# KRLGroup/gym-ma-survival-2d

Measured on NVIDIA B200. Metric: agent_steps_per_sec, higher is better.
Workload: dtype f32

## Files before the change

### gym-ma-survival-2d_b200/csrc/msv_abi.cu

```cuda
#include <cuda_runtime.h>
#include <math.h>
#include <stdio.h>
#include <stdlib.h>
#include <string.h>
#include <string>
#include <vector>
#include <map>
#include <algorithm>

#include "../../include/masurv.h"
#include "msv_launch.h"

extern "C" {
typedef struct { int32_t device_type; int32_t device_id; } DLDevice;
typedef struct { uint8_t code; uint8_t bits; uint16_t lanes; } DLDataType;
typedef struct {
  void* data; DLDevice device; int32_t ndim; DLDataType dtype;
  int64_t* shape; int64_t* strides; uint64_t byte_offset;
} DLTensor;
typedef struct DLManagedTensor {
  DLTensor dl_tensor; void* manager_ctx; void (*deleter)(struct DLManagedTensor*);
} DLManagedTensor;
}

// ... 1035 lines not shown
    const int64_t wr = 76 * A + 32 + 32 + 24 * PW + 16 + 8 + om + 4 * A + 1;
    return rd + wr;
  }
  if (which == 1) return 48 * A + 8 + om + 16 + 32 * B + 16 * B + 8 * H + 40 + (int64_t)h->obs.n_elems * 4;
  if (which == 2) return L > 0 ? 16 + 32 * B + 16 * B + 8 * H + 32 * A + 8 * A * L : 0;
  return 0;
}
int64_t msv_bytes_per_env_step(msv_handle* h) {
  return msv_kernel_bytes_per_env(h, 0) + msv_kernel_bytes_per_env(h, 1) + msv_kernel_bytes_per_env(h, 2);
}
int64_t msv_obs_bytes_per_env(msv_handle* h) { return h ? (int64_t)h->obs.n_elems * 4 : 0; }
int64_t msv_kernel_launches(msv_handle* h) { return h ? h->launches : 0; }
int msv_tile_plan(msv_handle* h, int32_t out[4]) {
  if (!h || !out) return MSV_ERR_INVALID;
  out[0] = h->C.epb; out[1] = h->C.N / h->C.epb; out[2] = h->C.epb * h->AC; out[3] = (h->handoff && h->cfg.auto_reset != 2) ? 1 : 0;
  return MSV_OK;
}

int msv_debug_profile(msv_handle* h, int enable, unsigned long long out[64]) {
  if (!h) return MSV_ERR_INVALID;
  DevGuard g(h->device); CK(cudaDeviceSynchronize());
  if (out) CK(msv_read_profile(out, 1));
  h->C.profile = enable;
  return MSV_OK;
}

int msv_debug_blocks(msv_handle* h, unsigned long long* out, int n_words) {
  if (!h || !out) return MSV_ERR_INVALID;
  DevGuard g(h->device); CK(cudaDeviceSynchronize());
  CK(msv_read_blocks(out, n_words));
  return MSV_OK;
}

int msv_debug_trace(msv_handle* h, unsigned long long* out, int n_words) {
  if (!h || !out) return MSV_ERR_INVALID;
  DevGuard g(h->device); CK(cudaDeviceSynchronize());
  CK(msv_read_trace(out, n_words));
  return MSV_OK;
}

void msv_philox4x32(const uint32_t ctr[4], const uint32_t key[2], uint32_t out[4]) {
  uint32_t c0 = ctr[0], c1 = ctr[1], c2 = ctr[2], c3 = ctr[3], k0 = key[0], k1 = key[1];
  for (int r = 0; r < 10; ++r) {
    uint64_t p0 = (uint64_t)0xD2511F53u * c0, p1 = (uint64_t)0xCD9E8D57u * c2;
    uint32_t n0 = (uint32_t)(p1 >> 32) ^ c1 ^ k0, n1 = (uint32_t)p1, n2 = (uint32_t)(p0 >> 32) ^ c3 ^ k1, n3 = (uint32_t)p0;
    c0 = n0; c1 = n1; c2 = n2; c3 = n3; k0 += 0x9E3779B9u; k1 += 0xBB67AE85u;
  }
  out[0] = c0; out[1] = c1; out[2] = c2; out[3] = c3;
}

}
```

### gym-ma-survival-2d_b200/csrc/msv_device.cuh

```cuda
#pragma once
#include <cuda_runtime.h>
#include <stdint.h>
#include <float.h>

#define DEV __device__ __forceinline__

#define B2_PI 3.14159265359f
#define B2_EPS FLT_EPSILON
#define B2_LINEAR_SLOP 0.005f
#define B2_POLY_RADIUS (2.0f * B2_LINEAR_SLOP)
#define B2_AABB_EXT 0.1f
#define B2_AABB_MULT 2.0f
#define B2_VEL_THRESHOLD 1.0f
#define B2_MAX_LIN_CORR 0.2f
#define B2_MAX_TRANSLATION 2.0f
#define B2_MAX_ROTATION (0.5f * B2_PI)
#define B2_BAUMGARTE 0.2f
#define B2_TOI_BAUMGARTE 0.75f
#define B2_TIME_TO_SLEEP 0.5f
#define B2_LIN_SLEEP_TOL 0.01f
#define B2_ANG_SLEEP_TOL (2.0f / 180.0f * B2_PI)
#define B2_MAX_SUBSTEPS 8

struct f2 { float x, y; };
// ... 290 lines not shown
  r.px = (1.0f - beta) * A.px + beta * A.px;
  r.py = (1.0f - beta) * A.py + beta * A.py;
  if (A.ang != 0.0f) {
    float angle = (1.0f - beta) * A.ang + beta * A.ang;
    if (angle != A.ang) rot_set(angle, r.qs, r.qc);
  }
  return r;
}
DEV f2 point_at(f2 c0, f2 c, float beta) { return vadd(vmul(1.0f - beta, c0), vmul(beta, c)); }

#define TOI_FAILED 1
#define TOI_OVERLAPPED 2
#define TOI_TOUCHING 3
#define TOI_SEPARATED 4

#ifdef MSV_CHECK
__device__ unsigned long long g_chk[2];
#define CHK(cond) do { if (!(cond)) { atomicAdd(&g_chk[0], 1ull); g_chk[1] = __LINE__; } } while (0)
__device__ __forceinline__ int chk_idx_(int i, int n, int line) {
  if ((unsigned)i < (unsigned)n) return i;
  atomicAdd(&g_chk[0], 1ull); g_chk[1] = (unsigned long long)line;
  return 0;
}
#define CHK_IDX(i, n) chk_idx_((i), (n), __LINE__)
#else
#define CHK(cond) do { } while (0)
#define CHK_IDX(i, n) (i)
#endif
#ifdef MSV_PROFILE
__device__ unsigned long long g_dbg[8];
__device__ unsigned long long g_cnt[16];
__device__ unsigned long long g_sub[16];
__device__ unsigned long long g_toi[16];
#define TOIPROF(x) x
#define SUB_BEGIN() long long sub_t_ = clock64()
#define SUB(k) do { long long n_ = clock64(); atomicAdd(&g_sub[k], (unsigned long long)(n_ - sub_t_)); sub_t_ = n_; } while (0)
#define SUBCNT(k, v) atomicAdd(&g_sub[k], (unsigned long long)(v))
#define SUBMAX(k, tag) atomicMax(&g_sub[k], ((unsigned long long)(clock64() - sub_t_) << 8) | (unsigned long long)((tag) & 255))
#define RARE_BEGIN() long long rare_t0_ = clock64()
#define RARE_END(k) do { atomicAdd(&g_cnt[2 * (k)], 1ull); atomicAdd(&g_cnt[2 * (k) + 1], (unsigned long long)(clock64() - rare_t0_)); } while (0)
#else
#define RARE_BEGIN() do { } while (0)
#define RARE_END(k) do { } while (0)
#define SUB_BEGIN() do { } while (0)
#define SUB(k) do { } while (0)
#define SUBCNT(k, v) do { } while (0)
#define SUBMAX(k, tag) do { } while (0)
#define TOIPROF(x)
#endif
struct ToiOut { int state; float t; };
__device__ __noinline__ ToiOut time_of_impact_v(const SBox A, f2 c0, f2 c, float rB) {
  int state = 0; float tOut = 1.0f;
  const float tMax = 1.0f;
#ifdef MSV_PROFILE
  long long dbg_t0 = clock64(); int dbg_roots = 0, dbg_push = 0;
#endif
  float totalRadius = B2_POLY_RADIUS + rB;
  float target = fmax_(B2_LINEAR_SLOP, totalRadius - 3.0f * B2_LINEAR_SLOP);
  float tolerance = 0.25f * B2_LINEAR_SLOP;
  float t1 = 0.0f;
  int iter = 0;
  {
    f2 l = sb_mulT(A, c0);
    float dx = fmax_(fabsf(l.x) - A.hx, 0.0f), dy = fmax_(fabsf(l.y) - A.hy, 0.0f);
    float d = sqrtf(dx * dx + dy * dy);
    if (d > 1e-3f && d < (target + tolerance) - 1e-3f) { ToiOut r0; r0.state = TOI_TOUCHING; r0.t = 0.0f; return r0; }
  }
  SimplexCache cache; cache.count = 0;
  for (;;) {
    const float t1_in = t1; const SimplexCache cache_in = cache;
    SBox xfA = box_at(A, t1); f2 pB = point_at(c0, c, t1);
    float distance = gjk_distance(cache, xfA, pB);
    if (distance <= 0.0f) { state = TOI_OVERLAPPED; tOut = 0.0f; break; }
    if (distance < target + tolerance) { state = TOI_TOUCHING; tOut = t1; break; }
    int ftype; f2 axis, localPoint = mk2(0.0f, 0.0f); int ptIndexA = 0;
    if (cache.count == 1) {
      ftype = 0; ptIndexA = cache.indexA[0];
      f2 pointA = sb_mul(xfA, sb_vert(xfA, cache.indexA[0]));
      axis = vsub(pB, pointA); vnormalize(axis);
    } else {
      ftype = 1;
      f2 lA1 = sb_vert(xfA, cache.indexA[0]), lA2 = sb_vert(xfA, cache.indexA[1]);
      axis = cross_vs(vsub(lA2, lA1), 1.0f); vnormalize(axis);
      f2 normal = qmul(xfA.qs, xfA.qc, axis);
      localPoint = vmul(0.5f, vadd(lA1, lA2));
      f2 pointA = sb_mul(xfA, localPoint);
      float s = vdot(vsub(pB, pointA), normal);
      if (s < 0.0f) axis = vneg(axis);
    }
    (void)ptIndexA;
    bool done = false;
    float t2 = tMax;
    int pushBackIter = 0;
    for (;;) {
      int indexA = -1; float s2;
      {
        SBox x2 = box_at(A, t2); f2 p2 = point_at(c0, c, t2);
        if (ftype == 0) {
          indexA = box_support(x2, qmulT(x2.qs, x2.qc, axis));
          f2 pointA = sb_mul(x2, sb_vert(x2, indexA));
          s2 = vdot(vsub(p2, pointA), axis);
        } else {
          f2 normal = qmul(x2.qs, x2.qc, axis);
          f2 pointA = sb_mul(x2, localPoint);
          s2 = vdot(vsub(p2, pointA), normal);
        }
      }
      if (s2 > target + tolerance) { state = TOI_SEPARATED; tOut = tMax; done = true; break; }
      if (s2 > target - tolerance) { t1 = t2; break; }
      auto evaluate = [&](float t) -> float {
        SBox xt = box_at(A, t); f2 pt = point_at(c0, c, t);
        if (ftype == 0) {
          f2 pointA = sb_mul(xt, sb_vert(xt, indexA));
          return vdot(vsub(pt, pointA), axis);
        }
        f2 normal = qmul(xt.qs, xt.qc, axis);
        f2 pointA = sb_mul(xt, localPoint);
        return vdot(vsub(pt, pointA), normal);
      };
      float s1 = evaluate(t1);
      if (s1 < target - tolerance) { state = TOI_FAILED; tOut = t1; done = true; break; }
      if (s1 <= target + tolerance) { state = TOI_TOUCHING; tOut = t1; done = true; break; }
      int rootIterCount = 0;
      float a1 = t1, a2 = t2;
      for (;;) {
        float t;
        if (rootIterCount & 1) t = a1 + (target - s1) * (a2 - a1) / (s2 - s1);
        else t = 0.5f * (a1 + a2);
        ++rootIterCount;
#ifdef MSV_PROFILE
        ++dbg_roots;
#endif
        float s = evaluate(t);
        if (fabsf(s - target) < tolerance) { t2 = t; break; }
        if (s > target) { a1 = t; s1 = s; } else { a2 = t; s2 = s; }
        if (rootIterCount == 50) break;
      }
      ++pushBackIter;
#ifdef MSV_PROFILE
      ++dbg_push;
#endif
      if (pushBackIter == 8) break;
    }
    ++iter;
    if (done) break;
    if (iter == 20) { state = TOI_FAILED; tOut = t1; break; }
    if (t1 == t1_in && cache.count == cache_in.count && cache.metric == cache_in.metric &&
        cache.indexA[0] == cache_in.indexA[0] && (cache.count < 2 || cache.indexA[1] == cache_in.indexA[1]) &&
        (cache.count < 3 || cache.indexA[2] == cache_in.indexA[2])) {
      state = TOI_FAILED; tOut = t1; break;
    }
  }
#ifdef MSV_PROFILE
  atomicAdd(&g_dbg[0], 1ull); atomicMax(&g_dbg[1], (unsigned long long)iter); atomicMax(&g_dbg[2], (unsigned long long)dbg_roots);
  atomicMax(&g_dbg[3], (unsigned long long)dbg_push); atomicMax(&g_dbg[4], (unsigned long long)(clock64() - dbg_t0));
  atomicAdd(&g_dbg[5], (unsigned long long)(clock64() - dbg_t0));
#endif
  ToiOut r; r.state = state; r.t = tOut;
  return r;
}
DEV int time_of_impact(const SBox& A, f2 c0, f2 c, float rB, float& tOut) {
  ToiOut r = time_of_impact_v(A, c0, c, rB);
  tOut = r.t; return r.state;
}

DEV void philox4x32(uint32_t c0, uint32_t c1, uint32_t c2, uint32_t c3,
                    uint32_t k0, uint32_t k1, uint32_t out[4]) {
#pragma unroll
  for (int r = 0; r < 10; ++r) {
    uint32_t hi0 = __umulhi(0xD2511F53u, c0), lo0 = 0xD2511F53u * c0;
    uint32_t hi1 = __umulhi(0xCD9E8D57u, c2), lo1 = 0xCD9E8D57u * c2;
    uint32_t n0 = hi1 ^ c1 ^ k0, n1 = lo1, n2 = hi0 ^ c3 ^ k1, n3 = lo0;
    c0 = n0; c1 = n1; c2 = n2; c3 = n3;
    k0 += 0x9E3779B9u; k1 += 0xBB67AE85u;
  }
  out[0] = c0; out[1] = c1; out[2] = c2; out[3] = c3;
}
```

### gym-ma-survival-2d_b200/csrc/msv_env.cuh

```cuda
#pragma once
#include "msv_device.cuh"
#include "msv_types.cuh"
#include "msv_launch.h"

enum { F_CX, F_CY, F_A, F_VX, F_VY, F_W, F_C0X, F_C0Y, F_A0, F_ALPHA0, F_SLEEP,
       F_FAT0, F_FAT1, F_FAT2, F_FAT3, F_FLAGS, F_QS, F_QC, F_COUNT };
enum { G_X, G_Y, G_HX, G_HY, G_AX, G_AY, G_ROT, G_F0, G_F1, G_F2, G_F3, G_COUNT };
enum { K_META, K_SEQ, K_MTYPE, K_LNX, K_LNY, K_LPX, K_LPY, K_NI, K_TI, K_NM, K_TM, K_COUNT };
enum { KS_NX = K_SEQ, KS_NY = K_MTYPE, KS_PX = K_LNX, KS_PY = K_LNY, KS_RBX = K_LPX, KS_RBY = K_LPY };

#define FL_ALIVE 1
#define FL_AWAKE 2
#define FL_ISLAND 4
#define FL_MOVED 8

#define KIND_NONE 0
#define KIND_AGENT 1
#define KIND_BOX 2
#define KIND_ITEM 3
#define KIND_HEAL 4
#define KIND_WALL 5

#define STREAM_SHUFFLE 0
#define STREAM_BOX 1
#define STREAM_ZONE 2
#define STREAM_DEATH 3

template <int AC, int BC> struct PairLayout {
  static constexpr int NAA = AC * (AC - 1) / 2;
  static constexpr int NAB = AC * BC;
  static constexpr int P = NAA + NAB + AC * 4;
  static constexpr int PW = (P + 63) / 64;
};

struct TCon {
  int p, seq;
  int a;
  int sid;
  int b;
  int flags;
  Manifold m;
  float ni, ti;
  f2 normal, rA, rB;
  float normalMass, tangentMass;
};

struct BodyS { f2 c; float a; f2 v; float w; float invM, invI; };

extern __shared__ float msv_sm[];


#ifndef MSV_INLINE_MASK
#define MSV_INLINE_MASK 0
#endif
#ifndef MSV_TOI_COOP
#define MSV_TOI_COOP 0
#endif
#ifndef MSV_FIXPOINT
#define MSV_FIXPOINT 1
#endif
#if (MSV_INLINE_MASK >> 0) & 1
#define COLD0 __device__ __forceinline__
#else
#define COLD0 __device__ __noinline__
#endif
#if (MSV_INLINE_MASK >> 1) & 1
#define COLD1 __device__ __forceinline__
#else
#define COLD1 __device__ __noinline__
#endif
#if (MSV_INLINE_MASK >> 2) & 1
#define COLD2 __device__ __forceinline__
#else
#define COLD2 __device__ __noinline__
#endif
#if (MSV_INLINE_MASK >> 3) & 1
#define COLD3 __device__ __forceinline__
#else
#define COLD3 __device__ __noinline__
#endif
#if (MSV_INLINE_MASK >> 4) & 1
#define COLD4 __device__ __forceinline__
#else
#define COLD4 __device__ __noinline__
#endif

__device__ __noinline__ double2 philox_uniform2_of(const DevConst& C, uint32_t genv, uint32_t episode, uint32_t step, uint32_t stream, uint32_t blk) {
  uint32_t o[4];
  philox4x32(genv, episode, step, (stream << 16) | blk, C.seed_lo, C.seed_hi, o);
// ... 31 lines not shown
    rec[MSV_SP_BOX + 4 * b + 2] = hx; rec[MSV_SP_BOX + 4 * b + 3] = hy;
  }
  for (int h = 0; h < C.H0; ++h) { const int cell = perm[--top]; rec[MSV_SP_HEAL + 2 * h] = C.grid_px[cell]; rec[MSV_SP_HEAL + 2 * h + 1] = C.grid_py[cell]; }
  for (int i = 0; i < C.A; ++i) { const int cell = perm[--top]; rec[MSV_SP_AGENT + 2 * i] = C.grid_px[cell]; rec[MSV_SP_AGENT + 2 * i + 1] = C.grid_py[cell]; }
  if (C.zone_centers_random) {
    int d = 0;
    for (int z = C.n_zones - 1; z >= 0; --z) {
      const double L = C.floor_size - 2 * C.zone_radiuses[z];
      const double2 uz = philox_uniform2_of(C, genv, episode, 0u, STREAM_ZONE, (uint32_t)(d >> 1)); d += 2;
      rec[MSV_SP_ZONE + 2 * z] = (float)((uz.x * L) - L / 2); rec[MSV_SP_ZONE + 2 * z + 1] = (float)((uz.y * L) - L / 2);
    }
  } else {
    for (int z = 0; z < C.n_zones; ++z) { rec[MSV_SP_ZONE + 2 * z] = (float)C.zone_centers[z][0]; rec[MSV_SP_ZONE + 2 * z + 1] = (float)C.zone_centers[z][1]; }
  }
}

template <int AC, int BC, int HC, int G>
struct Env {
  using PL = PairLayout<AC, BC>;
  static constexpr int P = PL::P, PW = PL::PW, NAA = PL::NAA;
  static constexpr int MAXC = AC <= 4 ? 16 : 24;
  enum { L_HEALTH = 0, L_CAUSE = L_HEALTH + AC, L_COOLDOWN = L_CAUSE + AC, L_INV = L_COOLDOWN + AC,
         L_SREW = L_INV + AC, L_SKILLS = L_SREW + AC, L_SEENA = L_SKILLS + AC, L_SEENX = L_SEENA + AC,
         L_KCAUSE = L_SEENX + AC, L_EPRET = L_KCAUSE + AC,
         L_NP = L_EPRET + AC, L_STEPS, L_EPISODE, L_BODYSEQ, L_CONTACTSEQ, L_FIRST, L_OVERFLOW, L_NEWFIX,
         L_ZX, L_ZY, L_ZR, L_ZPHASE, L_ZTCOOL, L_ZTSHRINK, L_ZEND,
         L_STSTEPS, L_STHEALS, L_STBOXES, L_STEPISODES, L_USEHEAL, L_USEBOX, L_NEWBOX,
         L_PREALIVE, L_DMASK, L_NKILLS, L_COUNT };
  static constexpr int SLOTS = AC / G;
  static constexpr int W_BOX = F_COUNT * AC, W_TC = W_BOX + G_COUNT * BC, W_MISC = W_TC + K_COUNT * MAXC;
  static constexpr int W_ITEM = W_MISC + 2, W_HEAL = W_ITEM + 2 * BC;
  static constexpr int W_LEAD = W_HEAL + 2 * HC;
  static constexpr int W_TOI = W_LEAD + L_COUNT;
  static constexpr int SM_USED = W_TOI + AC * (BC + 4);
  static constexpr int SM_WORDS = SM_USED + ((G - SM_USED % 32) + 32) % 32;
  static constexpr int NR = 3;
  static_assert(AC % G == 0 && G <= 32 && (G & (G - 1)) == 0, "G must be a power of two dividing AC");

  const DevConst& C;
  const DevState& S;
  int es, g, e, N;
  int sb;
  unsigned gmask;
  bool lead;

  int nb, ni, nh;
  unsigned long long ex[PW], tc[PW], en[PW];
  unsigned long long own[PW];
  int ntc;

  __device__ __forceinline__ Env(const DevConst& c, const DevState& s, int es_, int g_, unsigned gmask_, int e_)
      : C(c), S(s), es(es_), g(g_), e(e_), N(c.N), sb(es_ * SM_WORDS), gmask(gmask_), lead(g_ == 0) {
#pragma unroll
    for (int w = 0; w < PW; ++w) own[w] = 0ull;
    for (int i = g; i < AC; i += G) {
      for (int a = 0; a < i; ++a) setb(own, p_aa(a, i));
      for (int k = 0; k < BC; ++k) setb(own, p_ab(i, k));
      for (int k = 0; k < 4; ++k) setb(own, p_aw(i, k));
    }
  }

  DEV void gsync() const { __syncwarp(gmask); }
  template <class V> DEV V bc(V v) const { return __shfl_sync(gmask, v, 0, G); }
  template <class V> DEV V from(V v, int j) const { return __shfl_sync(gmask, v, j, G); }
  DEV unsigned or32(unsigned v) const {
#pragma unroll
    for (int o = 1; o < G; o <<= 1) v |= __shfl_xor_sync(gmask, v, o, G);
    return v;
// ... 7 lines not shown
  DEV void share_bits() {
#pragma unroll
    for (int w = 0; w < PW; ++w) { ex[w] = bc(ex[w]); tc[w] = bc(tc[w]); en[w] = bc(en[w]); }
  }
  DEV void merge_bits() {
#pragma unroll
    for (int w = 0; w < PW; ++w) { ex[w] = or64(ex[w] & own[w]); tc[w] = or64(tc[w] & own[w]); en[w] = or64(en[w] & own[w]); }
  }

  DEV void take(const Env& o) {
    nb = o.nb; ni = o.ni; nh = o.nh; ntc = o.ntc;
#pragma unroll
    for (int w = 0; w < PW; ++w) { ex[w] = o.ex[w]; tc[w] = o.tc[w]; en[w] = o.en[w]; }
  }
#define MSV_COLD(call) do { Env c_(*this); c_.call; take(c_); } while (0)
#ifndef MSV_INLINE_MASK
#define MSV_INLINE_MASK 0
#endif
#define MSV_COLDK(k, call) do { if ((MSV_INLINE_MASK >> (k)) & 1) { call; } else { Env c_(*this); c_.call; take(c_); } } while (0)

  DEV float& AG(int f, int i) { return msv_sm[sb + (CHK_IDX(f, F_COUNT) * AC + CHK_IDX(i, AC))]; }
  DEV int& AGF(int i) { return reinterpret_cast<int*>(msv_sm)[sb + (F_FLAGS * AC + CHK_IDX(i, AC))]; }
  DEV float& BX(int f, int k) { return msv_sm[sb + (W_BOX + CHK_IDX(f, G_COUNT) * BC + CHK_IDX(k, BC))]; }
  DEV int& BXROT(int k) { return reinterpret_cast<int*>(msv_sm)[sb + (W_BOX + G_ROT * BC + CHK_IDX(k, BC))]; }
  DEV float& KF(int f, int k) { return msv_sm[sb + (W_TC + CHK_IDX(f, K_COUNT) * MAXC + CHK_IDX(k, MAXC))]; }
  DEV int& KI(int f, int k) { return reinterpret_cast<int*>(msv_sm)[sb + (W_TC + CHK_IDX(f, K_COUNT) * MAXC + CHK_IDX(k, MAXC))]; }
  DEV int& NTC() { return reinterpret_cast<int*>(msv_sm)[sb + (W_MISC + 0)]; }
  DEV float& ITP(int c, int k) { return msv_sm[sb + (W_ITEM + CHK_IDX(c, 2) * BC + CHK_IDX(k, BC))]; }
  DEV float& HLP(int c, int k) { return msv_sm[sb + (W_HEAL + CHK_IDX(c, 2) * HC + CHK_IDX(k, HC))]; }
  DEV int& LI(int k) { return reinterpret_cast<int*>(msv_sm)[sb + (W_LEAD + CHK_IDX(k, L_COUNT))]; }
  DEV unsigned& LU(int k) { return reinterpret_cast<unsigned*>(msv_sm)[sb + (W_LEAD + CHK_IDX(k, L_COUNT))]; }
  DEV float& LF(int k) { return msv_sm[sb + (W_LEAD + CHK_IDX(k, L_COUNT))]; }
  DEV float& TOIA(int i, int k) { return msv_sm[sb + (W_TOI + CHK_IDX(i, AC) * (BC + 4) + CHK_IDX(k, BC + 4))]; }
  DEV int& OVF() { return reinterpret_cast<int*>(msv_sm)[sb + (W_MISC + 1)]; }
  DEV bool alive(int i) { return AGF(i) & FL_ALIVE; }
  DEV bool awake(int i) { return AGF(i) & FL_AWAKE; }
  DEV f2 apos(int i) { return mk2(AG(F_CX, i), AG(F_CY, i)); }
  DEV static int meta_pack(int p, int a, int sid, int b) { return p | ((a + 1) << 8) | ((sid < 0 ? 0 : sid) << 12) | (b << 16); }
  DEV static void meta_unpack(int m, int& p, int& a, int& sid, int& b) { p = m & 255; a = ((m >> 8) & 15) - 1; sid = (m >> 12) & 15; b = (m >> 16) & 15; }

  DEV static bool bit(const unsigned long long* m, int p) {
    unsigned long long w = m[0];
#pragma unroll
    for (int q = 1; q < PW; ++q) if ((p >> 6) == q) w = m[q];
    return (w >> (p & 63)) & 1ull;
  }
  DEV static void setb(unsigned long long* m, int p) {
#pragma unroll
    for (int q = 0; q < PW; ++q) if (PW == 1 || (p >> 6) == q) m[q] |= 1ull << (p & 63);
  }
  DEV static void clrb(unsigned long long* m, int p) {
#pragma unroll
    for (int q = 0; q < PW; ++q) if (PW == 1 || (p >> 6) == q) m[q] &= ~(1ull << (p & 63));
  }
  DEV static int p_aa(int i, int j) { return j * (j - 1) / 2 + i; }
  DEV static int p_ab(int i, int k) { return NAA + i * BC + k; }
  DEV static int p_aw(int i, int k) { return NAA + AC * BC + i * 4 + k; }
  DEV static void decode(int p, int& a, int& sid, int& b) {
    CHK((unsigned)p < (unsigned)P);
    if (p < NAA) {
      int j = 1; while (j * (j + 1) / 2 <= p) ++j;
      a = p - j * (j - 1) / 2; b = j; sid = -1;
    } else if (p < NAA + AC * BC) {
      int q = p - NAA; a = -1; b = q / BC; sid = q % BC;
    } else {
      int q = p - NAA - AC * BC; a = -1; b = q >> 2; sid = BC + (q & 3);
// ... 1140 lines not shown
        const f2 v_in = vB; const float w_in = wB; bool changed = false;
        for (int k = 0; k < nisl; ++k) {
          const float ni0 = KF(K_NI, k), ti0 = KF(K_TI, k);
          float ni_ = ni0, ti_ = ti0;
          solve_velocity_static(mk2(KF(KS_NX, k), KF(KS_NY, k)), mk2(KF(KS_RBX, k), KF(KS_RBY, k)), KF(K_NM, k), KF(K_TM, k), ni_, ti_, vB, wB);
          KF(K_NI, k) = ni_; KF(K_TI, k) = ti_;
          changed |= __float_as_uint(ni_) != __float_as_uint(ni0) || __float_as_uint(ti_) != __float_as_uint(ti0);
        }
        if (!changed && __float_as_uint(vB.x) == __float_as_uint(v_in.x) && __float_as_uint(vB.y) == __float_as_uint(v_in.y) &&
            __float_as_uint(wB) == __float_as_uint(w_in)) break;
      }
      AG(F_VX, b) = vB.x; AG(F_VY, b) = vB.y; AG(F_W, b) = wB;
    }
    SUB(3);
    integrate_position(b, subdt);
    AGF(b) &= ~FL_MOVED;
    synchronize_fixtures(b);
    if (AGF(b) & FL_MOVED) find_new_contacts_of(b);
    SUB(4);
    bool same = prevP == minP;
    auto snap = [&](int q, unsigned v) { if (SNAP(q) != v) same = false; SNAP(q) = v; };
    for (int f = 0; f < F_COUNT; ++f) snap(f, __float_as_uint(AG(f, b)));
#pragma unroll
    for (int w = 0; w < PW; ++w) {
      snap(F_COUNT + 6 * w + 0, (unsigned)ex[w]); snap(F_COUNT + 6 * w + 1, (unsigned)(ex[w] >> 32));
      snap(F_COUNT + 6 * w + 2, (unsigned)tc[w]); snap(F_COUNT + 6 * w + 3, (unsigned)(tc[w] >> 32));
      snap(F_COUNT + 6 * w + 4, (unsigned)en[w]); snap(F_COUNT + 6 * w + 5, (unsigned)(en[w] >> 32));
    }
    snap(SNAPW - 1, (unsigned)LI(L_CONTACTSEQ));
    SUB(5);
    return 1 | (same ? 2 : 0);
  }

  DEV void solve_toi(float dt) {
    static_assert(SLOTS == 1, "solve_toi: one agent per lane");
    const int i = g;
    if (i < C.A) { AGF(i) &= ~FL_ISLAND; AG(F_ALPHA0, i) = 0.0f; }
    unsigned long long evcnt = 0ull; unsigned cvalid = 0u;
    int prevP = -1;
    auto toi_alpha = [&](int j, int k) {
      const SBox sbx = static_box(k);
      const f2 q0 = mk2(AG(F_C0X, j), AG(F_C0Y, j)), q1 = apos(j);
      float beta = 1.0f;
      const int state = time_of_impact(sbx, q0, q1, C.agent_r, beta);
      const float alpha0 = AG(F_ALPHA0, j);
      return state == TOI_TOUCHING ? fmin_(alpha0 + (1.0f - alpha0) * beta, 1.0f) : 1.0f;
    };
    TOIPROF(long long tp0 = clock64(); long long tp_ev = 0; int tp_it = 0; int tp_ran = 0; int tp_not = 0; int tp_same = 0; int tp_calls = 0;)
    for (int guard = 0; guard < 64; ++guard) {
      TOIPROF(tp_it++;)
      unsigned need = 0u;
      int minP = -1, minSeq = -1; float minAlpha = 1.0f;
      auto consider = [&](int p, float alpha) {
        if (alpha < 1.0f) {
          const int sq = (int)S.pseq[p * N + e];
          if (alpha < minAlpha || (alpha == minAlpha && sq > minSeq)) { minAlpha = alpha; minP = p; minSeq = sq; }
        }
      };
      if (i < C.A && alive(i) && awake(i)) {
#pragma unroll
        for (int w = 0; w < PW; ++w) {
          unsigned long long mbits = ex[w] & en[w] & own[w];
          if (w == 0) mbits &= ~((1ull << NAA) - 1ull);
          while (mbits) {
            int p = w * 64 + __ffsll((long long)mbits) - 1; mbits &= mbits - 1;
            int a_, k, i_; decode(p, a_, k, i_);
            const int cnt = (int)((evcnt >> (4 * k)) & 15ull);
            if (cnt > C.toi_max_count) continue;
            if ((cvalid >> k) & 1u) { consider(p, TOIA(i, k)); continue; }
            const SBox sbx = static_box(k);
            const f2 l0 = sb_mulT(sbx, mk2(AG(F_C0X, i), AG(F_C0Y, i))), l1 = sb_mulT(sbx, apos(i));
            const float gx = fmax_(fmin_(l0.x, l1.x) - sbx.hx, -sbx.hx - fmax_(l0.x, l1.x));
            const float gy = fmax_(fmin_(l0.y, l1.y) - sbx.hy, -sbx.hy - fmax_(l0.y, l1.y));
            if (fmax_(gx, gy) > (B2_POLY_RADIUS + C.agent_r - 3.0f * B2_LINEAR_SLOP) + 0.25f * B2_LINEAR_SLOP + 0.004f) { TOIA(i, k) = 1.0f; cvalid |= 1u << k; }
            else if (MSV_TOI_COOP) need |= 1u << k;
            else { const float al = toi_alpha(i, k); TOIA(i, k) = al; cvalid |= 1u << k; consider(p, al); }
          }
        }
      }
      if (MSV_TOI_COOP && __any_sync(gmask, need != 0u)) {
        unsigned ms[G]; int T = 0;
#pragma unroll
        for (int j = 0; j < G; ++j) { ms[j] = from(need, j); T += __popc(ms[j]); }
        TOIPROF(tp_calls += T;)
        for (int r0 = 0; r0 < T; r0 += G) {
          const int t = r0 + g;
          int fj = -1, fk = 0, base = 0;
#pragma unroll
          for (int j = 0; j < G; ++j) {
            const int c = __popc(ms[j]);
            if (t >= base && t < base + c) { fj = j; fk = (int)__fns(ms[j], 0u, t - base + 1); }
            base += c;
          }
          if (fj >= 0) TOIA(fj, fk) = toi_alpha(fj, fk);
        }
        gsync();
        cvalid |= need;
        while (need) {
          const int k = __ffs((int)need) - 1; need &= need - 1u;
          consider(k < BC ? p_ab(i, k) : p_aw(i, k - BC), TOIA(i, k));
        }
      }
#pragma unroll
      for (int o = 1; o < G; o <<= 1) {
        float oa = __shfl_xor_sync(gmask, minAlpha, o, G);
        int op = __shfl_xor_sync(gmask, minP, o, G), os = __shfl_xor_sync(gmask, minSeq, o, G);
        if (op >= 0 && (oa < minAlpha || (oa == minAlpha && os > minSeq))) { minAlpha = oa; minP = op; minSeq = os; }
      }
      if (minP < 0 || 1.0f - 10.0f * B2_EPS < minAlpha) break;
      int ea, ek, eb; decode(minP, ea, ek, eb);
      const bool mine = eb == g;
      if (mine) cvalid &= ~(1u << ek);
      gsync();
      int r = 0;
      TOIPROF(long long tpe = clock64();)
      if (lead) {
        RARE_BEGIN();
        if ((MSV_INLINE_MASK >> 1) & 1) r = toi_event(minP, minAlpha, dt, prevP);
        else { Env c_(*this); r = c_.toi_event(minP, minAlpha, dt, prevP); take(c_); }
        if (r & 1) prevP = minP;
        RARE_END(1);
      }
      gsync();
      r = bc(r);
      TOIPROF(tp_ev += clock64() - tpe; if (r & 1) tp_ran++; else tp_not++; if (r & 2) tp_same++;)
      share_bits();
      if (mine) {
        const unsigned long long c4 = (evcnt >> (4 * ek)) & 15ull;
        if (c4 < 15ull) evcnt += 1ull << (4 * ek);
      }
      if (!(r & 1)) continue;
      if (mine) {
        if (r & 2) {
          const unsigned long long c4 = (evcnt >> (4 * ek)) & 15ull;
          if (c4 <= (unsigned long long)C.toi_max_count) evcnt = (evcnt & ~(15ull << (4 * ek))) | ((unsigned long long)(C.toi_max_count + 1) << (4 * ek));
        } else cvalid = 0u;
      }
    }
    gsync();
    TOIPROF(if (lead) { unsigned long long tot = (unsigned long long)(clock64() - tp0); unsigned long long old = atomicMax(&g_toi[0], tot);
      if (tot > old) { g_toi[1] = tp_it; g_toi[2] = tp_ran; g_toi[3] = tp_not; g_toi[4] = tp_same; g_toi[5] = (unsigned long long)tp_ev; g_toi[6] = tot - (unsigned long long)tp_ev; g_toi[7] = tp_calls; g_toi[8] = (unsigned long long)e; } })
  }

  __device__ __forceinline__ unsigned pre_motors(const uint8_t* actions, bool real) {
    unsigned flags = 0;
    for (int i = g; i < C.A; i += G) {
      int a0 = 1, a1 = 1, a2 = 1;
      if (real) {
        const uint8_t* a = actions + ((size_t)e * C.A + i) * 6;
        a0 = min((int)a[0], 2); a1 = min((int)a[1], 2); a2 = min((int)a[2], 2);
        flags |= (a[3] ? 1u : 0u) << i | (a[4] ? 1u : 0u) << (8 + i) | (a[5] ? 1u : 0u) << (16 + i);
      }
      if (!alive(i)) continue;
      float s, c; rot_set(AG(F_A, i), s, c);
      AG(F_QS, i) = s; AG(F_QC, i) = c;
      float par = C.imp_par[a0], nor = C.imp_nor[a1];
      float ix = c * par + (-s) * nor, iy = s * par + c * nor;
      wake(i);
      AG(F_VX, i) += C.inv_mass * ix; AG(F_VY, i) += C.inv_mass * iy;
      AG(F_W, i) += C.inv_I * C.imp_ang[a2];
    }
    return or32(flags);
  }
  DEV void pre_use_give(unsigned act) {
    LI(L_USEHEAL) = 0; LI(L_USEBOX) = 0; LI(L_NEWBOX) = 0;
    bool any = LI(L_NP) > 0;
#pragma unroll
    for (int i = 0; i < AC; ++i) if (i < C.A && (((act >> (8 + i)) | (act >> (16 + i))) & 1u) && (LI(L_INV + (i)) & 7) != 0 && alive(i)) any = true;
    if (any) { RARE_BEGIN(); MSV_COLDK(3, pre_use_give_body(act)); RARE_END(5); }
  }
  COLD3 void pre_use_give_body(unsigned act) {
    for (int q = 0; q < LI(L_NP); ++q) {
// ... 510 lines not shown
```

### gym-ma-survival-2d_b200/csrc/msv_kernels.cu

```cuda
#include <cstdlib>
#include "msv_env.cuh"
#include "msv_launch.h"

__device__ unsigned long long g_prof[64];
#ifdef MSV_PROFILE
#define MSV_BLK_MAX 2048
#define MSV_BLK_STAMPS 24
#define MSV_TR_MAX 4096
#define MSV_TR_ROWS 6
__device__ unsigned long long g_tr[2 * MSV_TR_ROWS * MSV_TR_MAX];
__device__ __forceinline__ unsigned long long gtime_ns() { unsigned long long t; asm volatile("mov.u64 %0, %%globaltimer;" : "=l"(t)); return t; }
#define TRACE(row, idx) do { if (threadIdx.x == 0 && (idx) < MSV_TR_MAX) g_tr[((C.tq_ticket & 1u) * MSV_TR_ROWS + (row)) * MSV_TR_MAX + (idx)] = gtime_ns(); } while (0)
__device__ unsigned long long g_blk[MSV_BLK_MAX * MSV_BLK_STAMPS];
#define BLK_STAMP() do { if (C.profile && threadIdx.x == 0 && blockIdx.x < MSV_BLK_MAX && blk_n < MSV_BLK_STAMPS) { g_blk[blockIdx.x * MSV_BLK_STAMPS + blk_n] = (unsigned long long)clock64(); blk_n++; } } while (0)
#define PROF(k) do { if (C.profile) { long long _t = clock64(); ph[k] += (unsigned long long)(_t - t_last); t_last = _t; } } while (0)
#define PROFW(k) do { if (C.profile) { long long _t = clock64(); wt[k] += (unsigned long long)(_t - t_last); t_last = _t; } } while (0)
#else
#define PROF(k) do { } while (0)
#define PROFW(k) do { } while (0)
#define BLK_STAMP() do { } while (0)
#define TRACE(row, idx) do { } while (0)
#endif

#define MSV_COLD_ON(env, call) do { if ((MSV_INLINE_MASK >> 4) & 1) { env.call; } else { auto c_ = env; c_.call; env.take(c_); } } while (0)
#ifndef MSV_SYNC_MASK_ALL
#define MSV_SYNC_MASK(G) ((G) >= 8 ? 0x3FF : 0x1F7)
#else
#define MSV_SYNC_MASK(G) (MSV_SYNC_MASK_ALL)
#endif
#ifdef MSV_NO_PHASE_SYNC
#define PHASE_SYNC(k) do { } while (0)
#else
#define PHASE_SYNC(k) do { if ((MSV_SYNC_MASK(G) >> (k)) & 1) __syncthreads(); PROFW(k); BLK_STAMP(); } while (0)
#endif
#define MSV_GROUP_SETUP(G)                                                                       \
  const int es = threadIdx.x / (G), g = threadIdx.x % (G);                                       \
  const int e = blockIdx.x * (blockDim.x / (G)) + es;   \
  const unsigned gmask = (((G) >= 32) ? 0xffffffffu : ((1u << (G)) - 1u)) << ((threadIdx.x & 31) & ~((G) - 1))

template <int AC, int BC, int HC, int G>
__global__ void __launch_bounds__(MSV_TPB)
k_step(const __grid_constant__ DevConst C, const __grid_constant__ DevState S,
       const __grid_constant__ DevOut Oc, const uint8_t* __restrict__ actions) {
  MSV_GROUP_SETUP(G);
  DevOut O = Oc;
  asm volatile("griddepcontrol.launch_dependents;" ::: "memory");
  if (C.pdl_wait) asm volatile("griddepcontrol.wait;" ::: "memory");
  TRACE(0, blockIdx.x);
  Env<AC, BC, HC, G> env(C, S, es, g, gmask, e);
#ifdef MSV_PROFILE
  long long t_last = C.profile ? clock64() : 0;
  const long long t_begin = t_last;
  unsigned long long ph[12] = {0, 0, 0, 0, 0, 0, 0, 0, 0, 0, 0, 0};
  unsigned long long wt[12] = {0, 0, 0, 0, 0, 0, 0, 0, 0, 0, 0, 0};
  int blk_n = 1;
  BLK_STAMP();
#endif
  env.load();
  const bool real = e < C.n_real;
  PROF(0);
  PHASE_SYNC(0);
  const unsigned act = env.pre_motors(actions, real);
  env.gsync();
  if (env.lead) env.pre_use_give(act);
  env.gsync();
  env.share_counts();
  const int newfix = env.bc(env.LI(env.L_NEWFIX));
  if (env.bc(env.LI(env.L_NEWBOX))) env.share_bits();
  PHASE_SYNC(6);
  env.pre_melee(act);
  PROF(1);
#pragma unroll 1
  for (int sub = 0; sub < 2; ++sub) {
    if (sub == 0 && newfix) { env.find_new_contacts(); env.LI(env.L_NEWFIX) = 0; }
    PROF(2);
    PHASE_SYNC(1);
    env.collide();
    PROF(3);
    PHASE_SYNC(2);
    const int first = env.bc(env.LI(env.L_FIRST));
    env.solve(C.dt, first ? 0.0f : C.dt_ratio1);
    PROF(4);
    PHASE_SYNC(9);
    env.solve_find_new();
    PROF(2);
    PHASE_SYNC(3);
    env.solve_toi(C.dt);
    env.LI(env.L_FIRST) = 0;
    PROF(5);
// ... 14 lines not shown
    PHASE_SYNC(7);
    if (env.lead) {
      bool done = env.rewards_done(O);
      if (done && C.auto_reset) {
        env.LI(env.L_STEPISODES)++;
        { RARE_BEGIN(); MSV_COLD_ON(env, reset()); RARE_END(2); }
        again = 1;
      }
      env.store_immune(O);
    }
    again = env.bc(again);
    if (!again) break;
    env.share_counts();
  }
  PROF(9);
  PHASE_SYNC(8);
  if (env.lead) env.store_obm();
  PROF(10);
  env.store();
  PROF(11);
  if (C.tq_ticket) {
    __syncthreads();
    if (threadIdx.x == 0) {
      const unsigned slot = atomicAdd(S.tq_tail, 1u) - C.tq_base;
      const unsigned long long v = ((unsigned long long)C.tq_ticket << 32) | (unsigned long long)blockIdx.x;
      asm volatile("st.release.gpu.global.u64 [%0], %1;" :: "l"(S.tq + slot), "l"(v) : "memory");
      TRACE(1, blockIdx.x);
    }
  }
#ifdef MSV_PROFILE
  __syncthreads();
  BLK_STAMP();
  if (C.profile && threadIdx.x == 0 && blockIdx.x < MSV_BLK_MAX) g_blk[blockIdx.x * MSV_BLK_STAMPS] = (unsigned long long)blk_n;
  if (C.profile && env.lead) {
    for (int k = 0; k < 12; ++k) { atomicAdd(&g_prof[k], ph[k]); atomicAdd(&g_prof[32 + k], wt[k]); }
    unsigned long long tot = (unsigned long long)(clock64() - t_begin);
    unsigned long long prev = atomicMax(&g_prof[12], tot);
    if (tot > prev) {
      for (int k = 0; k < 12; ++k) { g_prof[16 + k] = ph[k]; g_prof[48 + k] = wt[k]; }
      g_prof[13] = (unsigned long long)e;
    }
  }
#endif
}

template <int AC, int BC, int HC, int G>
__global__ void __launch_bounds__(MSV_TPB)
k_reset(const __grid_constant__ DevConst C, const __grid_constant__ DevState S,
        const __grid_constant__ DevOut Oc, int only_done) {
  MSV_GROUP_SETUP(G);
  DevOut O = Oc;
  if (only_done && !O.dones[e]) return;
  Env<AC, BC, HC, G> env(C, S, es, g, gmask, e);
  env.load();
  if (env.lead) {
    if (only_done) env.LI(env.L_STEPISODES)++;
    MSV_COLD_ON(env, reset());
  }
  env.share_counts();
  env.cameras();
  if (env.lead) {
    env.store_obm();
    env.store_immune(O);
    if (!only_done) {
      for (int i = 0; i < C.A; ++i) O.rewards[(size_t)e * C.A + i] = 0.0f;
      O.dones[e] = 0;
// ... 508 lines not shown
    default: *AC = 8; *BC = 8; *HC = 16; *P = PairLayout<8, 8>::P; *PW = PairLayout<8, 8>::PW; *sm_words = Env<8, 8, 16, 8>::SM_WORDS; break;
  }
}

cudaError_t msv_launch_stats(int N, int stride, int AC, float* sreward, int* skills, int4* smisc, double* out_reward,
                             unsigned long long* out_kills, unsigned long long* out_misc, cudaStream_t st) {
  k_stats<<<(N + 127) / 128, 128, 0, st>>>(N, stride, AC, sreward, skills, smisc, out_reward, out_kills, out_misc);
  return cudaPeekAtLastError();
}

cudaError_t msv_read_check(unsigned long long out[2]) {
#ifdef MSV_CHECK
  return cudaMemcpyFromSymbol(out, g_chk, sizeof(unsigned long long) * 2);
#else
  out[0] = ~0ull; out[1] = 0;
  return cudaSuccess;
#endif
}

cudaError_t msv_read_blocks(unsigned long long* out, int n_words) {
#ifdef MSV_PROFILE
  if (n_words > MSV_BLK_MAX * MSV_BLK_STAMPS) n_words = MSV_BLK_MAX * MSV_BLK_STAMPS;
  cudaError_t e_ = cudaMemcpyFromSymbol(out, g_blk, sizeof(unsigned long long) * (size_t)n_words);
  if (e_ == cudaSuccess && n_words >= MSV_BLK_MAX * MSV_BLK_STAMPS) {
    e_ = cudaMemcpyFromSymbol(out + (MSV_BLK_MAX - 1) * MSV_BLK_STAMPS, g_toi, sizeof(unsigned long long) * 16);
    unsigned long long z[16] = {0}; cudaMemcpyToSymbol(g_toi, z, sizeof z);
  }
  return e_;
#else
  (void)out; (void)n_words; return cudaErrorNotSupported;
#endif
}

cudaError_t msv_read_trace(unsigned long long* out, int n_words) {
#ifdef MSV_PROFILE
  if (n_words > 2 * MSV_TR_ROWS * MSV_TR_MAX) n_words = 2 * MSV_TR_ROWS * MSV_TR_MAX;
  cudaError_t e_ = cudaMemcpyFromSymbol(out, g_tr, sizeof(unsigned long long) * (size_t)n_words);
  if (e_ == cudaSuccess) { static unsigned long long z[2 * MSV_TR_ROWS * MSV_TR_MAX]; e_ = cudaMemcpyToSymbol(g_tr, z, sizeof z); }
  return e_;
#else
  (void)out; (void)n_words; return cudaErrorNotSupported;
#endif
}

cudaError_t msv_read_profile(unsigned long long out[64], int reset) {
  cudaError_t e = cudaMemcpyFromSymbol(out, g_prof, sizeof(unsigned long long) * 64);
  if (e != cudaSuccess) return e;
#ifdef MSV_PROFILE
  { unsigned long long d[8]; cudaMemcpyFromSymbol(d, g_dbg, sizeof d); out[28] = d[0]; out[29] = d[1]; out[30] = d[2]; out[31] = d[5]; unsigned long long z8[8] = {0}; if (reset) cudaMemcpyToSymbol(g_dbg, z8, sizeof z8); }
  { unsigned long long d[16]; cudaMemcpyFromSymbol(d, g_cnt, sizeof d); for (int k = 0; k < 4; ++k) out[44 + k] = 0; for (int k = 0; k < 16; ++k) if (k < 4) out[44 + k] = d[k]; 
    out[58] = d[4]; out[59] = d[5]; out[60] = d[6]; out[61] = d[7]; out[62] = d[8]; out[63] = d[9];
    out[14] = d[10]; out[15] = d[11]; out[42] = d[12]; out[43] = d[13];
    unsigned long long z16[16] = {0}; if (reset) cudaMemcpyToSymbol(g_cnt, z16, sizeof z16);
    unsigned long long sb_[16]; cudaMemcpyFromSymbol(sb_, g_sub, sizeof sb_);
    for (int k = 0; k < 6; ++k) out[20 + k] = sb_[k];
    for (int k = 0; k < 8; ++k) out[48 + k] = sb_[8 + k];
    out[26] = sb_[6]; out[27] = sb_[7];
    if (reset) cudaMemcpyToSymbol(g_sub, z16, sizeof z16); }
#endif
  if (reset) { unsigned long long z[64] = {0}; e = cudaMemcpyToSymbol(g_prof, z, sizeof z); }
  return e;
}
```

### gym-ma-survival-2d_b200/csrc/msv_launch.h

```cpp
#pragma once
#include "msv_types.cuh"
#ifndef MSV_TPB
#define MSV_TPB 512
#endif
cudaError_t msv_launch(int cap, int which, const DevConst& C, const DevState& S, const DevOut& O,
                       const uint8_t* actions, cudaStream_t st);
void msv_capacity(int cap, int* AC, int* BC, int* HC, int* P, int* PW, int* sm_words);
cudaError_t msv_launch_stats(int N, int stride, int AC, float* sreward, int* skills, int4* smisc, double* out_reward,
                             unsigned long long* out_kills, unsigned long long* out_misc, cudaStream_t st);
cudaError_t msv_read_profile(unsigned long long out[64], int reset);
cudaError_t msv_read_blocks(unsigned long long* out, int n_words);
cudaError_t msv_read_trace(unsigned long long* out, int n_words);
cudaError_t msv_read_check(unsigned long long out[2]);
cudaError_t msv_launch_spare(const DevConst& C, const DevState& S, const uint8_t* dones, int only_done, cudaStream_t st);
cudaError_t msv_launch_obs(const DevConst& C, const DevState& S, const ObsTable& T, int AC, const uint8_t* only_if, cudaStream_t st);
cudaError_t msv_launch_lidar(const DevConst& C, const DevState& S, const DevOut& O, int BC, int HC, cudaStream_t st);
struct RenderArgs {
  int first, count, H, W, BC, HC, lidar;
  int TW, TR, tiles_x, tiles_per_img;
  float s, half_floor;
  uint8_t* out;
};
cudaError_t msv_launch_render(const DevConst& C, const DevState& S, const DevOut& O, RenderArgs R, cudaStream_t st);
int msv_palette(uint8_t* out_rgb, int capacity);
```

Before: 614.7 million.

## Precompute first-pass TOI calls block-wide with cross-warp job redistribution

Before the TOI event loop, each agent culls its static-box candidates and collects the ones needing a full time-of-impact solve. These jobs are compacted per warp into shared memory and spread evenly across all threads of the block, so divergent TOI work no longer serialises on a few lanes. The old optional group-cooperative path is removed. Profiling counters for TOI outcomes are also added. The cost is extra block-wide syncs, more shared memory for job slots, and work on pairs that the later loop might not need.

```diff
diff --git a/gym-ma-survival-2d_b200/csrc/msv_abi.cu b/gym-ma-survival-2d_b200/csrc/msv_abi.cu
--- a/gym-ma-survival-2d_b200/csrc/msv_abi.cu
+++ b/gym-ma-survival-2d_b200/csrc/msv_abi.cu
@@ -1091,6 +1091,13 @@
   return MSV_OK;
 }
 
+int msv_debug_toi_census(msv_handle* h, unsigned long long* out, int n_words) {
+  if (!h || !out) return MSV_ERR_INVALID;
+  DevGuard g(h->device); CK(cudaDeviceSynchronize());
+  CK(msv_read_toi_census(out, n_words));
+  return MSV_OK;
+}
+
 int msv_debug_trace(msv_handle* h, unsigned long long* out, int n_words) {
   if (!h || !out) return MSV_ERR_INVALID;
   DevGuard g(h->device); CK(cudaDeviceSynchronize());
diff --git a/gym-ma-survival-2d_b200/csrc/msv_device.cuh b/gym-ma-survival-2d_b200/csrc/msv_device.cuh
--- a/gym-ma-survival-2d_b200/csrc/msv_device.cuh
+++ b/gym-ma-survival-2d_b200/csrc/msv_device.cuh
@@ -346,6 +346,9 @@
 __device__ unsigned long long g_cnt[16];
 __device__ unsigned long long g_sub[16];
 __device__ unsigned long long g_toi[16];
+#define MSV_TOIC_WORDS 32
+__device__ unsigned long long g_toic[MSV_TOIC_WORDS];
+__device__ unsigned g_toiblk[2048 * 4];
 #define TOIPROF(x) x
 #define SUB_BEGIN() long long sub_t_ = clock64()
 #define SUB(k) do { long long n_ = clock64(); atomicAdd(&g_sub[k], (unsigned long long)(n_ - sub_t_)); sub_t_ = n_; } while (0)
@@ -367,7 +370,7 @@
   int state = 0; float tOut = 1.0f;
   const float tMax = 1.0f;
 #ifdef MSV_PROFILE
-  long long dbg_t0 = clock64(); int dbg_roots = 0, dbg_push = 0;
+  long long dbg_t0 = clock64(); int dbg_roots = 0, dbg_push = 0, dbg_gjk = 0, dbg_r50 = 0, dbg_rep50 = 0; bool dbg_stuck = false;
 #endif
   float totalRadius = B2_POLY_RADIUS + rB;
   float target = fmax_(B2_LINEAR_SLOP, totalRadius - 3.0f * B2_LINEAR_SLOP);
@@ -378,13 +381,21 @@
     f2 l = sb_mulT(A, c0);
     float dx = fmax_(fabsf(l.x) - A.hx, 0.0f), dy = fmax_(fabsf(l.y) - A.hy, 0.0f);
     float d = sqrtf(dx * dx + dy * dy);
-    if (d > 1e-3f && d < (target + tolerance) - 1e-3f) { ToiOut r0; r0.state = TOI_TOUCHING; r0.t = 0.0f; return r0; }
+    if (d > 1e-3f && d < (target + tolerance) - 1e-3f) {
+#ifdef MSV_PROFILE
+      atomicAdd(&g_toic[0], 1ull); atomicAdd(&g_toic[1], (unsigned long long)(clock64() - dbg_t0));
+#endif
+      ToiOut r0; r0.state = TOI_TOUCHING; r0.t = 0.0f; return r0;
+    }
   }
   SimplexCache cache; cache.count = 0;
   for (;;) {
     const float t1_in = t1; const SimplexCache cache_in = cache;
     SBox xfA = box_at(A, t1); f2 pB = point_at(c0, c, t1);
     float distance = gjk_distance(cache, xfA, pB);
+#ifdef MSV_PROFILE
+    ++dbg_gjk;
+#endif
     if (distance <= 0.0f) { state = TOI_OVERLAPPED; tOut = 0.0f; break; }
     if (distance < target + tolerance) { state = TOI_TOUCHING; tOut = t1; break; }
     int ftype; f2 axis, localPoint = mk2(0.0f, 0.0f); int ptIndexA = 0;
@@ -406,6 +417,9 @@
     bool done = false;
     float t2 = tMax;
     int pushBackIter = 0;
+#ifdef MSV_PROFILE
+    dbg_stuck = false;
+#endif
     for (;;) {
       int indexA = -1; float s2;
       {
@@ -448,7 +462,13 @@
         float s = evaluate(t);
         if (fabsf(s - target) < tolerance) { t2 = t; break; }
         if (s > target) { a1 = t; s1 = s; } else { a2 = t; s2 = s; }
-        if (rootIterCount == 50) break;
+        if (rootIterCount == 50) {
+#ifdef MSV_PROFILE
+          ++dbg_r50; if (dbg_stuck) ++dbg_rep50;
+          dbg_stuck = true;
+#endif
+          break;
+        }
       }
       ++pushBackIter;
 #ifdef MSV_PROFILE
@@ -469,6 +489,13 @@
   atomicAdd(&g_dbg[0], 1ull); atomicMax(&g_dbg[1], (unsigned long long)iter); atomicMax(&g_dbg[2], (unsigned long long)dbg_roots);
   atomicMax(&g_dbg[3], (unsigned long long)dbg_push); atomicMax(&g_dbg[4], (unsigned long long)(clock64() - dbg_t0));
   atomicAdd(&g_dbg[5], (unsigned long long)(clock64() - dbg_t0));
+  {
+    const int oc = state == TOI_SEPARATED ? 1 : state == TOI_TOUCHING ? (tOut < 1.0f ? 2 : 3) : state == TOI_FAILED ? 4 : 5;
+    atomicAdd(&g_toic[2 * oc], 1ull); atomicAdd(&g_toic[2 * oc + 1], (unsigned long long)(clock64() - dbg_t0));
+    atomicAdd(&g_toic[12], (unsigned long long)dbg_gjk); atomicAdd(&g_toic[13], (unsigned long long)dbg_push); atomicAdd(&g_toic[14], (unsigned long long)dbg_roots);
+    atomicMax(&g_toic[15], (unsigned long long)dbg_gjk); atomicMax(&g_toic[16], (unsigned long long)dbg_push); atomicMax(&g_toic[17], (unsigned long long)dbg_roots);
+    atomicAdd(&g_toic[18], (unsigned long long)dbg_r50); atomicAdd(&g_toic[19], (unsigned long long)dbg_rep50);
+  }
 #endif
   ToiOut r; r.state = state; r.t = tOut;
   return r;
diff --git a/gym-ma-survival-2d_b200/csrc/msv_env.cuh b/gym-ma-survival-2d_b200/csrc/msv_env.cuh
--- a/gym-ma-survival-2d_b200/csrc/msv_env.cuh
+++ b/gym-ma-survival-2d_b200/csrc/msv_env.cuh
@@ -52,9 +52,6 @@
 
 #ifndef MSV_INLINE_MASK
 #define MSV_INLINE_MASK 0
-#endif
-#ifndef MSV_TOI_COOP
-#define MSV_TOI_COOP 0
 #endif
 #ifndef MSV_FIXPOINT
 #define MSV_FIXPOINT 1
@@ -152,8 +149,11 @@
   static constexpr int W_ITEM = W_MISC + 2, W_HEAL = W_ITEM + 2 * BC;
   static constexpr int W_LEAD = W_HEAL + 2 * HC;
   static constexpr int W_TOI = W_LEAD + L_COUNT;
-  static constexpr int SM_USED = W_TOI + AC * (BC + 4);
+  static constexpr int W_JOB = W_TOI + AC * (BC + 4);
+  static constexpr int SM_USED = W_JOB + 8;
   static constexpr int SM_WORDS = SM_USED + ((G - SM_USED % 32) + 32) % 32;
+  static constexpr int JOBW = SM_WORDS - W_JOB;
+  static constexpr int WJOBS = JOBW * (32 / G) - 1 < 32 ? JOBW * (32 / G) - 1 : 32;
   static constexpr int NR = 3;
   static_assert(AC % G == 0 && G <= 32 && (G & (G - 1)) == 0, "G must be a power of two dividing AC");
 
@@ -227,6 +227,7 @@
   DEV unsigned& LU(int k) { return reinterpret_cast<unsigned*>(msv_sm)[sb + (W_LEAD + CHK_IDX(k, L_COUNT))]; }
   DEV float& LF(int k) { return msv_sm[sb + (W_LEAD + CHK_IDX(k, L_COUNT))]; }
   DEV float& TOIA(int i, int k) { return msv_sm[sb + (W_TOI + CHK_IDX(i, AC) * (BC + 4) + CHK_IDX(k, BC + 4))]; }
+  DEV static int& JOB(int ws, int r) { r = CHK_IDX(r, WJOBS + 1); return reinterpret_cast<int*>(msv_sm)[(ws + r / JOBW) * SM_WORDS + W_JOB + r % JOBW]; }
   DEV int& OVF() { return reinterpret_cast<int*>(msv_sm)[sb + (W_MISC + 1)]; }
   DEV bool alive(int i) { return AGF(i) & FL_ALIVE; }
   DEV bool awake(int i) { return AGF(i) & FL_AWAKE; }
@@ -1433,24 +1434,94 @@
     return 1 | (same ? 2 : 0);
   }
 
+#ifdef MSV_PROFILE
+  int tp_sub = 0;
+  DEV void toi_census(int c) {
+    const unsigned sum = __reduce_add_sync(0xffffffffu, (unsigned)c), mx = __reduce_max_sync(0xffffffffu, (unsigned)c);
+    const int sub = tp_sub++;
+    if ((threadIdx.x & 31) == 0 && blockIdx.x < 2048 && sub < 2 && C.profile) {
+      atomicAdd(&g_toiblk[blockIdx.x * 4 + 2 * sub], sum); atomicMax(&g_toiblk[blockIdx.x * 4 + 2 * sub + 1], mx);
+    }
+  }
+#endif
+
+  DEV bool toi_culled(int i, int k) {
+    const SBox sbx = static_box(k);
+    const f2 l0 = sb_mulT(sbx, mk2(AG(F_C0X, i), AG(F_C0Y, i))), l1 = sb_mulT(sbx, apos(i));
+    const float gx = fmax_(fmin_(l0.x, l1.x) - sbx.hx, -sbx.hx - fmax_(l0.x, l1.x));
+    const float gy = fmax_(fmin_(l0.y, l1.y) - sbx.hy, -sbx.hy - fmax_(l0.y, l1.y));
+    return fmax_(gx, gy) > (B2_POLY_RADIUS + C.agent_r - 3.0f * B2_LINEAR_SLOP) + 0.25f * B2_LINEAR_SLOP + 0.004f;
+  }
+  DEV float toi_alpha(int j, int k) {
+    const SBox sbx = static_box(k);
+    const f2 q0 = mk2(AG(F_C0X, j), AG(F_C0Y, j)), q1 = apos(j);
+    float beta = 1.0f;
+    const int state = time_of_impact(sbx, q0, q1, C.agent_r, beta);
+    const float alpha0 = AG(F_ALPHA0, j);
+    return state == TOI_TOUCHING ? fmin_(alpha0 + (1.0f - alpha0) * beta, 1.0f) : 1.0f;
+  }
+
+  DEV void toi_pass(unsigned need) {
+    const int lane = threadIdx.x & 31, ws = (threadIdx.x >> 5) * (32 / G);
+    do {
+      unsigned rest = need;
+      need = 0u;
+      int n = 0;
+      for (unsigned b; (b = __ballot_sync(0xffffffffu, rest != 0u)) != 0u; n += __popc(b)) {
+        if (rest) {
+          const int k = __ffs((int)rest) - 1, r = n + __popc(b & ((1u << lane) - 1u));
+          rest &= rest - 1u;
+          if (r < WJOBS) JOB(ws, 1 + r) = (int)threadIdx.x | k << 16;
+          else need |= 1u << k;
+        }
+      }
+      if (lane == 0) JOB(ws, 0) = min(n, WJOBS);
+      __syncthreads();
+      const int t = threadIdx.x, c = lane < (int)(blockDim.x >> 5) ? JOB(lane * (32 / G), 0) : 0;
+      int incl = c;
+#pragma unroll
+      for (int o = 1; o < 32; o <<= 1) { const int v = __shfl_up_sync(0xffffffffu, incl, o); if (lane >= o) incl += v; }
+      int w = 0;
+#pragma unroll
+      for (int h = 16; h; h >>= 1)
+        if (__shfl_sync(0xffffffffu, incl, w + h - 1) <= t) w += h;
+      const int first = __shfl_sync(0xffffffffu, incl - c, w);
+      if (t < __shfl_sync(0xffffffffu, incl, 31)) {
+        const int jb = JOB(w * (32 / G), 1 + t - first), jt = jb & 0xffff, jk = jb >> 16;
+        Env o(*this);
+        o.sb = jt / G * SM_WORDS;
+        o.TOIA(jt % G, jk) = o.toi_alpha(jt % G, jk);
+      }
+    } while (__syncthreads_or(need != 0u));
+  }
+
   DEV void solve_toi(float dt) {
     static_assert(SLOTS == 1, "solve_toi: one agent per lane");
     const int i = g;
     if (i < C.A) { AGF(i) &= ~FL_ISLAND; AG(F_ALPHA0, i) = 0.0f; }
     unsigned long long evcnt = 0ull; unsigned cvalid = 0u;
     int prevP = -1;
-    auto toi_alpha = [&](int j, int k) {
-      const SBox sbx = static_box(k);
-      const f2 q0 = mk2(AG(F_C0X, j), AG(F_C0Y, j)), q1 = apos(j);
-      float beta = 1.0f;
-      const int state = time_of_impact(sbx, q0, q1, C.agent_r, beta);
-      const float alpha0 = AG(F_ALPHA0, j);
-      return state == TOI_TOUCHING ? fmin_(alpha0 + (1.0f - alpha0) * beta, 1.0f) : 1.0f;
-    };
     TOIPROF(long long tp0 = clock64(); long long tp_ev = 0; int tp_it = 0; int tp_ran = 0; int tp_not = 0; int tp_same = 0; int tp_calls = 0;)
+    {
+      unsigned need = 0u;
+      if (i < C.A && alive(i) && awake(i)) {
+#pragma unroll
+        for (int w = 0; w < PW; ++w) {
+          unsigned long long mbits = ex[w] & en[w] & own[w];
+          if (w == 0) mbits &= ~((1ull << NAA) - 1ull);
+          while (mbits) {
+            int p = w * 64 + __ffsll((long long)mbits) - 1; mbits &= mbits - 1;
+            int a_, k, i_; decode(p, a_, k, i_);
+            if (toi_culled(i, k)) TOIA(i, k) = 1.0f;
+            else need |= 1u << k;
+          }
+        }
+      }
+      TOIPROF(tp_calls = __popc(need); toi_census(tp_calls);)
+      toi_pass(need);
+    }
     for (int guard = 0; guard < 64; ++guard) {
       TOIPROF(tp_it++;)
-      unsigned need = 0u;
       int minP = -1, minSeq = -1; float minAlpha = 1.0f;
       auto consider = [&](int p, float alpha) {
         if (alpha < 1.0f) {
@@ -1468,38 +1539,11 @@
             int a_, k, i_; decode(p, a_, k, i_);
             const int cnt = (int)((evcnt >> (4 * k)) & 15ull);
             if (cnt > C.toi_max_count) continue;
+            if (guard == 0) cvalid |= 1u << k;
             if ((cvalid >> k) & 1u) { consider(p, TOIA(i, k)); continue; }
-            const SBox sbx = static_box(k);
-            const f2 l0 = sb_mulT(sbx, mk2(AG(F_C0X, i), AG(F_C0Y, i))), l1 = sb_mulT(sbx, apos(i));
-            const float gx = fmax_(fmin_(l0.x, l1.x) - sbx.hx, -sbx.hx - fmax_(l0.x, l1.x));
-            const float gy = fmax_(fmin_(l0.y, l1.y) - sbx.hy, -sbx.hy - fmax_(l0.y, l1.y));
-            if (fmax_(gx, gy) > (B2_POLY_RADIUS + C.agent_r - 3.0f * B2_LINEAR_SLOP) + 0.25f * B2_LINEAR_SLOP + 0.004f) { TOIA(i, k) = 1.0f; cvalid |= 1u << k; }
-            else if (MSV_TOI_COOP) need |= 1u << k;
+            if (toi_culled(i, k)) { TOIA(i, k) = 1.0f; cvalid |= 1u << k; }
             else { const float al = toi_alpha(i, k); TOIA(i, k) = al; cvalid |= 1u << k; consider(p, al); }
           }
-        }
-      }
-      if (MSV_TOI_COOP && __any_sync(gmask, need != 0u)) {
-        unsigned ms[G]; int T = 0;
-#pragma unroll
-        for (int j = 0; j < G; ++j) { ms[j] = from(need, j); T += __popc(ms[j]); }
-        TOIPROF(tp_calls += T;)
-        for (int r0 = 0; r0 < T; r0 += G) {
-          const int t = r0 + g;
-          int fj = -1, fk = 0, base = 0;
-#pragma unroll
-          for (int j = 0; j < G; ++j) {
-            const int c = __popc(ms[j]);
-            if (t >= base && t < base + c) { fj = j; fk = (int)__fns(ms[j], 0u, t - base + 1); }
-            base += c;
-          }
-          if (fj >= 0) TOIA(fj, fk) = toi_alpha(fj, fk);
-        }
-        gsync();
-        cvalid |= need;
-        while (need) {
-          const int k = __ffs((int)need) - 1; need &= need - 1u;
-          consider(k < BC ? p_ab(i, k) : p_aw(i, k - BC), TOIA(i, k));
         }
       }
 #pragma unroll
@@ -1539,6 +1583,7 @@
       }
     }
     gsync();
+    TOIPROF(for (int o = 1; o < G; o <<= 1) tp_calls = max(tp_calls, __shfl_xor_sync(gmask, tp_calls, o, G));)
     TOIPROF(if (lead) { unsigned long long tot = (unsigned long long)(clock64() - tp0); unsigned long long old = atomicMax(&g_toi[0], tot);
       if (tot > old) { g_toi[1] = tp_it; g_toi[2] = tp_ran; g_toi[3] = tp_not; g_toi[4] = tp_same; g_toi[5] = (unsigned long long)tp_ev; g_toi[6] = tot - (unsigned long long)tp_ev; g_toi[7] = tp_calls; g_toi[8] = (unsigned long long)e; } })
   }
diff --git a/gym-ma-survival-2d_b200/csrc/msv_kernels.cu b/gym-ma-survival-2d_b200/csrc/msv_kernels.cu
--- a/gym-ma-survival-2d_b200/csrc/msv_kernels.cu
+++ b/gym-ma-survival-2d_b200/csrc/msv_kernels.cu
@@ -55,6 +55,8 @@
   unsigned long long wt[12] = {0, 0, 0, 0, 0, 0, 0, 0, 0, 0, 0, 0};
   int blk_n = 1;
   BLK_STAMP();
+  if (C.profile && threadIdx.x < 4 && blockIdx.x < 2048) g_toiblk[blockIdx.x * 4 + threadIdx.x] = 0u;
+  __syncthreads();
 #endif
   env.load();
   const bool real = e < C.n_real;
@@ -135,6 +137,14 @@
   __syncthreads();
   BLK_STAMP();
   if (C.profile && threadIdx.x == 0 && blockIdx.x < MSV_BLK_MAX) g_blk[blockIdx.x * MSV_BLK_STAMPS] = (unsigned long long)blk_n;
+  if (C.profile && threadIdx.x == 0 && blockIdx.x < 2048) {
+    for (int s = 0; s < 2; ++s) {
+      const unsigned calls = atomicAdd(&g_toiblk[blockIdx.x * 4 + 2 * s], 0u), lane = atomicAdd(&g_toiblk[blockIdx.x * 4 + 2 * s + 1], 0u);
+      unsigned long long* r = g_toic + 20 + 6 * s;
+      atomicAdd(&r[0], 1ull); atomicAdd(&r[1], (unsigned long long)calls); atomicMax(&r[2], (unsigned long long)calls);
+      atomicAdd(&r[3], (unsigned long long)lane); atomicMax(&r[4], (unsigned long long)lane);
+    }
+  }
   if (C.profile && env.lead) {
     for (int k = 0; k < 12; ++k) { atomicAdd(&g_prof[k], ph[k]); atomicAdd(&g_prof[32 + k], wt[k]); }
     unsigned long long tot = (unsigned long long)(clock64() - t_begin);
@@ -709,6 +719,17 @@
 #endif
 }
 
+cudaError_t msv_read_toi_census(unsigned long long* out, int n_words) {
+#ifdef MSV_PROFILE
+  if (n_words > MSV_TOIC_WORDS) n_words = MSV_TOIC_WORDS;
+  cudaError_t e_ = cudaMemcpyFromSymbol(out, g_toic, sizeof(unsigned long long) * (size_t)n_words);
+  if (e_ == cudaSuccess) { unsigned long long z[MSV_TOIC_WORDS] = {0}; e_ = cudaMemcpyToSymbol(g_toic, z, sizeof z); }
+  return e_;
+#else
+  (void)out; (void)n_words; return cudaErrorNotSupported;
+#endif
+}
+
 cudaError_t msv_read_trace(unsigned long long* out, int n_words) {
 #ifdef MSV_PROFILE
   if (n_words > 2 * MSV_TR_ROWS * MSV_TR_MAX) n_words = 2 * MSV_TR_ROWS * MSV_TR_MAX;
diff --git a/gym-ma-survival-2d_b200/csrc/msv_launch.h b/gym-ma-survival-2d_b200/csrc/msv_launch.h
--- a/gym-ma-survival-2d_b200/csrc/msv_launch.h
+++ b/gym-ma-survival-2d_b200/csrc/msv_launch.h
@@ -11,6 +11,7 @@
 cudaError_t msv_read_profile(unsigned long long out[64], int reset);
 cudaError_t msv_read_blocks(unsigned long long* out, int n_words);
 cudaError_t msv_read_trace(unsigned long long* out, int n_words);
+cudaError_t msv_read_toi_census(unsigned long long* out, int n_words);
 cudaError_t msv_read_check(unsigned long long out[2]);
 cudaError_t msv_launch_spare(const DevConst& C, const DevState& S, const uint8_t* dones, int only_done, cudaStream_t st);
 cudaError_t msv_launch_obs(const DevConst& C, const DevState& S, const ObsTable& T, int AC, const uint8_t* only_if, cudaStream_t st);
```

Measured after the change: 578.9 million (median of 6 runs). 0.942x the previous value.
